# De-Rosa/PPO-BipedalWalker

Measured on NVIDIA B200. Metric: walker env-steps/sec (SAT physics step), higher is better.
Workload: dtype f32

## Files before the change

ppo-bipedalwalker_b200/csrc/physics_lanes.cu:

```cuda
#include <cstdio>
#include <cstdlib>
#include "physics.cuh"
#include "physics_math.cuh"

#ifndef WB_SAT_UNROLL
#define WB_SAT_UNROLL 6
#endif

namespace wb {
namespace pl {
constexpr int kSatUnroll = WB_SAT_UNROLL;

constexpr unsigned kFull = 0xFFFFFFFFu;

#ifdef WB_PHASE_PROFILE
__device__ unsigned long long g_prof[24];
__device__ __forceinline__ long long prof_clock() {
  long long t;
  asm volatile("mov.u64 %0, %%clock64;" : "=l"(t)::"memory");
  return t;
}
__device__ long long g_prof_sat_scratch;
#endif


__constant__ Material c_materials[WB_MAX_MATERIALS];
__constant__ float c_init_state[kStateFloats];
__constant__ FloorConst c_floor;

enum { LLL = 0, LLU = 1, BODY = 2, RLL = 3, RLU = 4, FLOOR = 5 };

constexpr int kV2Cen = 30;
constexpr int kV2Vel = 35;
constexpr int kV2Count = 40;
constexpr int kFOmega = 0;
constexpr int kFAngle = 5;
constexpr int kFCount = 10;

__device__ __forceinline__ int nverts(int b) { return b == BODY ? 5 : 6; }

template <int L_, int E_>
struct Env {
  static constexpr int L = L_;
  static constexpr int E = E_;
  float2* v2;
  float* f;
  const FloorConst* fl;
  int sub;
  int gsub;
  int gshift;
  int col;
  bool live;
  int flags;
  float im_w;
  float ii_pole;
  float e_ww, mu_ww, e_wf, mu_wf;
};

template <class EV> __device__ __forceinline__ float2& V2(const EV& e, int slot) { return e.v2[slot * EV::E]; }
template <class EV> __device__ __forceinline__ float& F1(const EV& e, int slot) { return e.f[slot * EV::E]; }
template <class EV> __device__ __forceinline__ float inv_inertia(const EV& e, int b) { return b == BODY ? 0.0003f : e.ii_pole; }
template <class EV> __device__ __forceinline__ void set_materials(EV& e, const Material& mw, const Material& mf) {
  e.im_w = mw.inverse_mass;
  e.ii_pole = fmul(0.001f, mw.inverse_mass);
  e.e_ww = net_max(mw.restitution, mw.restitution);
  e.mu_ww = net_min(mw.friction, mw.friction);
  e.e_wf = net_max(mw.restitution, mf.restitution);
  e.mu_wf = net_min(mw.friction, mf.friction);
}
template <int L> __device__ __forceinline__ void lanes_sync() { if (L > 1) __syncwarp(); }
template <class EV, int G> __device__ __forceinline__ bool group_any(const EV& e, bool pred) {
  if (EV::L == 1) return pred;
  const unsigned b = __ballot_sync(kFull, pred);
  return ((b >> e.gshift) & ((1u << G) - 1u)) != 0u;
}

struct BodyDyn {
  float2 c, v;
  float w, im, ii;
};

template <class EV> __device__ __forceinline__ BodyDyn load_dyn(const EV& e, int b) {
  BodyDyn d;
  d.c = V2(e, kV2Cen + b);
  d.v = V2(e, kV2Vel + b);
  d.w = F1(e, kFOmega + b);
  d.im = e.im_w;
  d.ii = inv_inertia(e, b);
  return d;
}
template <class EV> __device__ __forceinline__ BodyDyn floor_dyn(const EV& e) {
  BodyDyn d;
  d.c = e.fl->cen;
  d.v = mk2(0.0f, 0.0f);
  d.w = 0.0f;
  d.im = 0.0f;
  d.ii = 0.0f;
  return d;
}
template <class EV> __device__ __forceinline__ void store_dyn(const EV& e, int b, const BodyDyn& d) {
  V2(e, kV2Vel + b) = d.v;
  F1(e, kFOmega + b) = d.w;
}

__device__ __forceinline__ void calculate_impulse(const BodyDyn& A, const BodyDyn& B, float2 contact, float force, float2 n,
                                                  float2& rA, float2& rB, float& impulse) {
  rA = vsub(contact, A.c);
  const float2 perpA = mk2(-rA.y, rA.x);
  const float kA = vdot(n, perpA);
  rB = vsub(contact, B.c);
  const float2 perpB = mk2(-rB.y, rB.x);
  const float kB = vdot(n, perpB);
  const float2 va = vadd(A.v, vmul(perpA, A.w));
  const float2 vb = vadd(B.v, vmul(perpB, B.w));
  const float2 vrel = vsub(vb, va);
  const float vn = vdot(vrel, n);
  const float j = fmul(-force, vn);
  const float2 k = mk2(kA, kB);
  const float2 kki = vmul2_nosum(vmul2_nosum(k, k), mk2(A.ii, B.ii));
  const float denom = fadd(fadd(fadd(A.im, B.im), kki.x), kki.y);
  impulse = fdiv(j, denom);
}

__device__ __forceinline__ void apply_impulses(BodyDyn& A, BodyDyn& B, float2 n, float impulse, float2 rA, float2 rB) {
  const float2 J = vmul(n, impulse);
  const float2 velA = vsub(A.v, vmul(J, A.im));
  const float2 velB = vadd(B.v, vmul(J, B.im));
  const float2 perpA = mk2(-rA.y, rA.x);
  const float wA = fsub(A.w, fmul(vdot(perpA, J), A.ii));
  const float2 perpB = mk2(-rB.y, rB.x);
  const float wB = fadd(B.w, fmul(vdot(perpB, J), B.ii));
  A.v = velA;
  B.v = velB;
  A.w = wA;
  B.w = wB;
}

template <class EV, int G>
__device__ __forceinline__ void move_bodies(const EV& e, bool on, int A, float2 dA, bool moveB, int B, float2 dB) {
#pragma unroll
  for (int it0 = 0; it0 < 14; it0 += G) {
    const int it = it0 + e.gsub;
    const bool second = it >= 7;
    const int k = second ? it - 7 : it;
    const int b = second ? B : A;
    if (on && it < 14 && (!second || moveB)) {
      const int slot = (k < 6) ? b * 6 + k : kV2Cen + b;
      V2(e, slot) = vadd(V2(e, slot), second ? dB : dA);
    }
  }
}

template <class EV, bool TRACE, int G = EV::L>
__device__ __forceinline__ void joint_step(const EV& e, int A, int ia, int B, int ib, wb_joint_trace* tr) {
  const bool leader = (G == EV::L) ? e.sub == 0 : e.gsub == 0;
  const float2 pA = V2(e, A * 6 + ia);
  const float2 pB = V2(e, B * 6 + ib);
  float2 ab = vsub(pB, pA);
  const float depth = fsqrt(vdot(ab, ab));
  if (TRACE) {
    if (tr && e.live && leader) {
      tr->active = !(depth < 0.1f);
      tr->depth = depth;
    }
  }
  const bool active = e.live && !(depth < 0.1f);
  if (!__any_sync(kFull, active)) return;
  ab = vnormalize_fast(ab);
  const float2 dA = vhalf(vmul(ab, depth));
  const float2 dB = vhalf(vmul(vneg(ab), depth));
  BodyDyn X = load_dyn(e, B);
  BodyDyn Y = load_dyn(e, A);
  lanes_sync<EV::L>();
  move_bodies<EV, G>(e, active, A, dA, true, B, dB);
  X.c = vadd(X.c, dB);
  Y.c = vadd(Y.c, dA);
  const float2 contact = vhalf(vadd(vadd(pA, dA), vadd(pB, dB)));
  float2 rX, rY;
  float j;
  calculate_impulse(X, Y, contact, fadd(1.0f, 1.0f), ab, rX, rY, j);
  apply_impulses(X, Y, ab, j, rX, rY);
  if (active && leader) {
    store_dyn(e, B, X);
    store_dyn(e, A, Y);
  }
  lanes_sync<EV::L>();
}

__device__ __forceinline__ void project6(const float2 (&P)[6], float2 ax, float& mn, float& mx) {
  const float t0 = vdot(ax, P[0]), t1 = vdot(ax, P[1]), t2 = vdot(ax, P[2]);
  const float t3 = vdot(ax, P[3]), t4 = vdot(ax, P[4]), t5 = vdot(ax, P[5]);
  mn = fminf(fminf(fminf(FLT_MAX, t0), fminf(t1, t2)), fminf(fminf(t3, t4), t5));
  mx = fmaxf(fmaxf(fmaxf(-FLT_MAX, t0), fmaxf(t1, t2)), fmaxf(fmaxf(t3, t4), t5));
}
__device__ __forceinline__ void project4(const float2* P, float2 ax, float& mn, float& mx) {
  const float t0 = vdot(ax, P[0]), t1 = vdot(ax, P[1]), t2 = vdot(ax, P[2]), t3 = vdot(ax, P[3]);
  mn = fminf(fminf(fminf(FLT_MAX, t0), t1), fminf(t2, t3));
  mx = fmaxf(fmaxf(fmaxf(-FLT_MAX, t0), t1), fmaxf(t2, t3));
}

struct Face {
  float2 a, b, max;
};

__device__ __forceinline__ Face face_from(float2 sv, float2 next, float2 prev, float2 nrm) {
  const float2 after = vnormalize_fast(vsub(sv, next));
  const float2 before = vnormalize_fast(vsub(sv, prev));
  const bool use_before = vdot(nrm, before) >= vdot(nrm, after);
  Face f;
  f.a = use_before ? sv : next;
  f.b = use_before ? prev : sv;
  f.max = sv;
  return f;
}

__device__ __forceinline__ int support_index6(const float2 (&P)[6], float2 nrm) {
  float best = FLT_MAX;
  int k = 0;
#pragma unroll
  for (int i = 0; i < 6; i++) {
    const float pr = vdot(P[i], nrm);
    const bool lt = pr < best;
    k = lt ? i : k;
    best = lt ? pr : best;
  }
  return k;
}

template <class EV>
__device__ __forceinline__ Face significant_face_body(const EV& e, int b, const float2 (&P)[6], float2 nrm) {
  const int n = nverts(b);
  const int k = support_index6(P, nrm);
  const int kn = (k + 1 == n) ? 0 : k + 1;
  const int kp = (k == 0) ? n - 1 : k - 1;
  return face_from(V2(e, b * 6 + k), V2(e, b * 6 + kn), V2(e, b * 6 + kp), nrm);
}

template <class EV>
__device__ __forceinline__ Face significant_face_floor(const EV& e, float2 nrm) {
  float best = FLT_MAX;
  int k = 0;
#pragma unroll
  for (int i = 0; i < 4; i++) {
    const float pr = vdot(e.fl->v[i], nrm);
    const bool lt = pr < best;
    k = lt ? i : k;
    best = lt ? pr : best;
  }
  return face_from(e.fl->v[k], e.fl->v[(k + 1) & 3], e.fl->v[(k + 3) & 3], nrm);
}

__device__ __forceinline__ int clip_vectors(float2 a, float2 b, float2 nrm, float offset, float2& o0, float2& o1) {
  int cnt = 0;
  const float2 dab = vsub(mk2(vdot(a, nrm), vdot(b, nrm)), mk2(offset, offset));
  const float da = dab.x, db = dab.y;
  if (da >= 0.0f) {
    o0 = a;
    cnt = 1;
  }
  if (db >= 0.0f) {
    if (cnt == 0) o0 = b; else o1 = b;
    cnt++;
  }
  if (fmul(da, db) < 0.0f) {
    float2 ed = vsub(b, a);
    const float location = fdiv(da, fsub(da, db));
    ed = vmul(ed, location);
    ed = vadd(ed, a);
    if (cnt == 0) o0 = ed; else if (cnt == 1) o1 = ed;
    cnt++;
  }
  return cnt;
}

__device__ __forceinline__ bool veq(float2 a, float2 b) { return a.x == b.x && a.y == b.y; }

__device__ __forceinline__ int contact_points(Face ref, Face inc, float2 normal, float2& c0, float2& c1) {
  float2 rf = vsub(ref.b, ref.a);
  const float2 ifv = vsub(inc.b, inc.a);
  if (fabsf(vdot(rf, normal)) > fabsf(vdot(ifv, normal))) {
    const Face t = ref;
    ref = inc;
    inc = t;
    rf = vsub(ref.b, ref.a);
  }
  rf = vnormalize_fast(rf);
  float offset = vdot(rf, ref.a);
  float2 p0 = mk2(0.f, 0.f), p1 = mk2(0.f, 0.f);
  int cnt = clip_vectors(inc.a, inc.b, rf, offset, p0, p1);
  if (cnt < 2) return 0;
  offset = vdot(rf, ref.b);
  float2 q0 = mk2(0.f, 0.f), q1 = mk2(0.f, 0.f);
  cnt = clip_vectors(p0, p1, vneg(rf), -offset, q0, q1);
  if (cnt < 2) return 0;
  cnt = 2;
  const float2 rn = mk2(rf.y, -rf.x);
  const float maximum = vdot(rn, ref.max);
  if (fsub(vdot(rn, q0), maximum) < 0.0f) {
    q0 = q1;
    cnt = 1;
  }
  const float2 last = (cnt == 2) ? q1 : q0;
  if (fsub(vdot(rn, last), maximum) < 0.0f) {
    if (cnt == 2) {
      if (veq(q0, q1)) q0 = q1;
      cnt = 1;
    } else {
      cnt = 0;
    }
  }
  c0 = q0;
  c1 = q1;
  return cnt;
}

__device__ __forceinline__ void resolve_impulses(BodyDyn& X, BodyDyn& Y, int ncp, float2 c0, float2 c1, float2 normal, float e, float mu) {
  const float2 contact = (ncp == 2) ? vhalf(vadd(c0, c1)) : c0;
  const float2 tangent = mk2(-normal.y, normal.x);
  float2 rA, rB, rAf, rBf;
  float j, jf;
  calculate_impulse(X, Y, contact, fadd(1.0f, e), normal, rA, rB, j);
  calculate_impulse(X, Y, contact, mu, tangent, rAf, rBf, jf);
  apply_impulses(X, Y, normal, j, rA, rB);
  apply_impulses(X, Y, tangent, jf, rAf, rBf);
}

__device__ __forceinline__ void resolve_impulses_split(BodyDyn& X, BodyDyn& Y, int ncp, float2 c0, float2 c1, float2 normal, float e, float mu,
                                                       bool odd) {
  const float2 contact = (ncp == 2) ? vhalf(vadd(c0, c1)) : c0;
  const float2 tangent = mk2(-normal.y, normal.x);
  float2 rA, rB;
  float mine;
  calculate_impulse(X, Y, contact, odd ? mu : fadd(1.0f, e), odd ? tangent : normal, rA, rB, mine);
  const float other = __shfl_xor_sync(kFull, mine, 1);
  apply_impulses(X, Y, normal, odd ? other : mine, rA, rB);
  apply_impulses(X, Y, tangent, odd ? mine : other, rA, rB);
}

__device__ __forceinline__ void aabb6(const float2 (&P)[6], float2& mn, float2& mx) {
  mn.x = fminf(fminf(fminf(P[0].x, P[1].x), fminf(P[2].x, P[3].x)), fminf(P[4].x, P[5].x));
  mn.y = fminf(fminf(fminf(P[0].y, P[1].y), fminf(P[2].y, P[3].y)), fminf(P[4].y, P[5].y));
  mx.x = fmaxf(fmaxf(fmaxf(P[0].x, P[1].x), fmaxf(P[2].x, P[3].x)), fmaxf(P[4].x, P[5].x));
  mx.y = fmaxf(fmaxf(fmaxf(P[0].y, P[1].y), fmaxf(P[2].y, P[3].y)), fmaxf(P[4].y, P[5].y));
}
__device__ __forceinline__ bool aabb_hit(float2 amin, float2 amax, float2 bmin, float2 bmax) {
  return amin.x < bmax.x && amax.x > bmin.x && amin.y < bmax.y && amax.y > bmin.y;
}

#ifndef WB_SHARED_CONTACTS
#define WB_SHARED_CONTACTS 0
#endif
}
namespace pc {
template <int G, int kE> __device__ __forceinline__ void group_env_by_col(pl::Env<G, kE>& e, int col, bool live);
}
namespace pl {
template <class EV, int G>
__device__ __noinline__ void contact_stage_shared(int col, bool live, bool colliding, int A, int B, bool floorb, float depth, int idx, float2 normal) {
  static_assert(G > 1, "two or more lanes per pair");
  EV e;
  pc::group_env_by_col<G, EV::E>(e, col, live);
  const FloorConst& fl = *e.fl;
#pragma unroll
  for (int m = 1; m < G; m <<= 1) {
    const float od = __shfl_xor_sync(kFull, depth, m);
    const int oi = __shfl_xor_sync(kFull, idx, m);
    const float ox = __shfl_xor_sync(kFull, normal.x, m);
    const float oy = __shfl_xor_sync(kFull, normal.y, m);
    if (od < depth || (od == depth && oi < idx)) {
      depth = od;
      idx = oi;
      normal = mk2(ox, oy);
    }
  }
  BodyDyn X = load_dyn(e, A);
  BodyDyn Y = load_dyn(e, floorb ? A : B);
  if (floorb) Y = floor_dyn(e);
  if (vdot(vsub(Y.c, X.c), normal) > 0.0f) normal = vmul(normal, -1.0f);
  const bool odd = (e.gsub & 1) != 0;
  const float2 nn = odd ? vneg(normal) : normal;
  const bool mine_floor = odd && floorb;
  const float2* vb = mine_floor ? fl.v : &V2(e, (odd ? B : A) * 6);
  const int stride = mine_floor ? 1 : EV::E;
  const int n = mine_floor ? 4 : nverts(odd ? B : A);
  float2 P[6];
#pragma unroll
  for (int i = 0; i < 6; i++) P[i] = vb[((mine_floor && i >= 4) ? 0 : i) * stride];
  const int k = support_index6(P, nn);
  const int kn = (k + 1 == n) ? 0 : k + 1;
  const int kp = (k == 0) ? n - 1 : k - 1;
  const Face mine = face_from(vb[k * stride], vb[kn * stride], vb[kp * stride], nn);
  Face other;
  other.a.x = __shfl_xor_sync(kFull, mine.a.x, 1);
  other.a.y = __shfl_xor_sync(kFull, mine.a.y, 1);
  other.b.x = __shfl_xor_sync(kFull, mine.b.x, 1);
  other.b.y = __shfl_xor_sync(kFull, mine.b.y, 1);
  other.max.x = __shfl_xor_sync(kFull, mine.max.x, 1);
  other.max.y = __shfl_xor_sync(kFull, mine.max.y, 1);
  const Face ref = odd ? other : mine;
  const Face inc = odd ? mine : other;
  float2 c0 = mk2(0.f, 0.f), c1 = mk2(0.f, 0.f);
  const int ncp = contact_points(ref, inc, normal, c0, c1);
  const float2 dA = floorb ? vmul(normal, depth) : vhalf(vmul(normal, depth));
  const float2 dB = floorb ? mk2(0.f, 0.f) : vhalf(vmul(vneg(normal), depth));
  lanes_sync<EV::L>();
  move_bodies<EV, G>(e, colliding, A, dA, !floorb, B, dB);
  X.c = vadd(X.c, dA);
  if (!floorb) Y.c = vadd(Y.c, dB);
  resolve_impulses_split(X, Y, ncp, c0, c1, normal, floorb ? e.e_wf : e.e_ww, floorb ? e.mu_wf : e.mu_ww, odd);
  if (ncp > 0 && colliding && e.gsub == 0) {
    store_dyn(e, A, X);
    if (!floorb) store_dyn(e, B, Y);
  }
  lanes_sync<EV::L>();
}

template <class EV, int G, bool TRACE, bool FLOORB, int VOTE = -1, bool KNOWN_HIT = false, bool SHARED_CONTACTS = false>
__device__ __forceinline__ void resolve_pair(EV& e, bool want, int A, int B, wb_pair_trace* tr, int* sep_axis = nullptr) {
  const FloorConst& fl = *e.fl;
  float2 PA[6], PB[6];
#pragma unroll
  for (int i = 0; i < 6; i++) PA[i] = V2(e, A * 6 + i);
  if (!FLOORB) {
#pragma unroll
    for (int i = 0; i < 6; i++) PB[i] = V2(e, B * 6 + i);
  }
  bool hit = want;
  if (!KNOWN_HIT) {
    float2 amin, amax, bmin, bmax;
    aabb6(PA, amin, amax);
    if (FLOORB) {
      bmin = fl.bb_min;
      bmax = fl.bb_max;
    } else {
      aabb6(PB, bmin, bmax);
    }
    hit = want && aabb_hit(amin, amax, bmin, bmax);
  }
  if (FLOORB && hit) e.flags |= (1 << A);
  wb_pair_trace rec;
  if (TRACE) {
    rec.other = FLOORB ? FLOOR : B;
    rec.aabb = hit ? 1 : 0;
    rec.sat = 0;
    rec.axis = -1;
    rec.nx = rec.ny = rec.depth = 0.0f;
    rec.ncontacts = 0;
    rec.c0x = rec.c0y = rec.c1x = rec.c1y = 0.0f;
  }
#ifdef WB_PHASE_PROFILE
  const long long rp_t0 = prof_clock();
  long long rp_t1 = rp_t0;
#endif
  bool colliding = false;
  if (__any_sync(kFull, hit)) {
    const int nA = nverts(A);
    float depth = FLT_MAX;
    float2 normal = mk2(0.0f, 0.0f);
    int idx = 0x7FFFFFFF;
    bool sep = false;
    constexpr bool kVote = VOTE < 0 ? (G != 4) : (VOTE != 0);
    bool my_sep = false;
    auto accumulate = [&](bool use, float2 axis, int axis_idx, float omin, float omax, float tmin, float tmax) {
      const float2 dd = vsub(mk2(tmax, omax), mk2(omin, tmin));
      const float temp = fminf(dd.x, dd.y);
      const bool overlapping = (omin < tmax) && (tmin < omax);
      if (use && temp < depth) {
        depth = temp;
        normal = axis;
        idx = axis_idx;
      }
      if (sep_axis != nullptr && use && !overlapping && !sep && !my_sep) *sep_axis = axis_idx;
      if (!kVote) {
        my_sep = my_sep || (use && !overlapping);
        return false;
      }
      const bool separated = group_any<EV, G>(e, use && !overlapping);
      sep = sep || separated;
      return !__any_sync(kFull, hit && !sep);
    };
    auto edge_axis = [&](int own, int k, bool& skip) {
      const float2 p0 = V2(e, own * 6 + k), p1 = V2(e, own * 6 + (k == 5 ? 0 : k + 1));
      const float2 edge = vsub(p1, p0);
      const float2 axis = mk2(-edge.y, edge.x);
      skip = (axis.x == 0.0f) && (axis.y == 0.0f);
      return vnormalize_fast(axis);
    };
    auto edge_axis_reg = [&](const float2 (&P)[6], int r, bool odd, bool& skip) {
      const float2 p0 = odd ? P[(r + 1) % 6] : P[r % 6], p1 = odd ? P[(r + 2) % 6] : P[(r + 1) % 6];
      const float2 edge = vsub(p1, p0);
      const float2 axis = mk2(-edge.y, edge.x);
      skip = (axis.x == 0.0f) && (axis.y == 0.0f);
      return vnormalize_fast(axis);
    };
    auto round_a_vs_floor = [&](int r) {
      const int i = r + e.gsub;
      const bool valid = i < 6;
      bool skip;
      const float2 axis = (G == 2 && !kVote) ? edge_axis_reg(PA, r, e.gsub != 0, skip) : edge_axis(A, valid ? i : 0, skip);
      float omin, omax, tmin, tmax;
      project6(PA, axis, omin, omax);
      project4(fl.v, axis, tmin, tmax);
      return accumulate(valid && !skip, axis, i, omin, omax, tmin, tmax);
    };
    auto round_floor_vs_a = [&](int r) {
      const int i = r + e.gsub;
      const bool valid = i < 4;
      const int k = valid ? i : 0;
      const float2 axis = fl.axis[k];
      float tmin, tmax;
      project6(PA, axis, tmin, tmax);
      return accumulate(valid && fl.skip[k] == 0, axis, nA + k, fl.pmin[k], fl.pmax[k], tmin, tmax);
    };
    auto round_pole = [&](int r) {
      const int i = r + e.gsub;
      const bool valid = i < 12;
      const bool ownA = i < 6;
      const int k = ownA ? i : (valid ? i - 6 : 0);
      bool skip;
      float2 axis;
      if (G == 2 && !kVote) {
        axis = (r < 6) ? edge_axis_reg(PA, r, e.gsub != 0, skip) : edge_axis_reg(PB, r - 6, e.gsub != 0, skip);
      } else {
        axis = edge_axis(ownA ? A : B, k, skip);
      }
      float amn, amx, bmn, bmx;
      project6(PA, axis, amn, amx);
      project6(PB, axis, bmn, bmx);
      return accumulate(valid && !skip, axis, ownA ? i : nA + k, amn, amx, bmn, bmx);
    };
    if (kVote) {
      if (FLOORB) {
        bool done = false;
#pragma unroll 1
        for (int r = 0; r < 6 && !done; r += G) done = round_a_vs_floor(r);
#pragma unroll 1
        for (int r = 0; r < 4 && !done; r += G) done = round_floor_vs_a(r);
      } else {
#pragma unroll 1
        for (int r = 0; r < 12; r += G)
          if (round_pole(r)) break;
      }
    } else {
      if (FLOORB) {
#pragma unroll kSatUnroll
        for (int r = 0; r < 6; r += G) round_a_vs_floor(r);
#pragma unroll kSatUnroll
        for (int r = 0; r < 4; r += G) round_floor_vs_a(r);
      } else {
#pragma unroll kSatUnroll
        for (int r = 0; r < 12; r += G) round_pole(r);
      }
      sep = group_any<EV, G>(e, my_sep);
    }
    colliding = hit && !sep;
#ifdef WB_PHASE_PROFILE
    rp_t1 = prof_clock();
#endif
    if constexpr (SHARED_CONTACTS && G > 1 && !TRACE) {
      if (__any_sync(kFull, colliding)) contact_stage_shared<EV, G>(e.col, e.live, colliding, A, B, FLOORB, depth, idx, normal);
    } else if (__any_sync(kFull, colliding)) {
      if (G > 1) {
#pragma unroll
        for (int m = 1; m < G; m <<= 1) {
          const float od = __shfl_xor_sync(kFull, depth, m);
          const int oi = __shfl_xor_sync(kFull, idx, m);
          const float ox = __shfl_xor_sync(kFull, normal.x, m);
          const float oy = __shfl_xor_sync(kFull, normal.y, m);
          if (od < depth || (od == depth && oi < idx)) {
            depth = od;
            idx = oi;
            normal = mk2(ox, oy);
          }
        }
      }
      BodyDyn X = load_dyn(e, A);
      BodyDyn Y = FLOORB ? floor_dyn(e) : load_dyn(e, B);
      if (vdot(vsub(Y.c, X.c), normal) > 0.0f) normal = vmul(normal, -1.0f);
      Face ref, inc;
      if (G == 1) {
        ref = significant_face_body(e, A, PA, normal);
        inc = FLOORB ? significant_face_floor(e, vneg(normal)) : significant_face_body(e, B, PB, vneg(normal));
      } else {
        const bool odd = (e.gsub & 1) != 0;
        const float2 nn = odd ? vneg(normal) : normal;
        float2 P[6];
        int n, stride;
        const float2* vb;
        if (FLOORB) {
#pragma unroll
          for (int i = 0; i < 6; i++) {
            const float2 f = fl.v[i < 4 ? i : 0];
            P[i] = odd ? f : PA[i];
          }
          n = odd ? 4 : nA;
          vb = odd ? fl.v : &V2(e, A * 6);
          stride = odd ? 1 : EV::E;
        } else {
#pragma unroll
          for (int i = 0; i < 6; i++) P[i] = odd ? PB[i] : PA[i];
          n = nverts(odd ? B : A);
          vb = &V2(e, (odd ? B : A) * 6);
          stride = EV::E;
        }
        const int k = support_index6(P, nn);
        const int kn = (k + 1 == n) ? 0 : k + 1;
        const int kp = (k == 0) ? n - 1 : k - 1;
        const Face mine = face_from(vb[k * stride], vb[kn * stride], vb[kp * stride], nn);
        Face other;
        other.a.x = __shfl_xor_sync(kFull, mine.a.x, 1);
        other.a.y = __shfl_xor_sync(kFull, mine.a.y, 1);
        other.b.x = __shfl_xor_sync(kFull, mine.b.x, 1);
        other.b.y = __shfl_xor_sync(kFull, mine.b.y, 1);
        other.max.x = __shfl_xor_sync(kFull, mine.max.x, 1);
        other.max.y = __shfl_xor_sync(kFull, mine.max.y, 1);
        ref = odd ? other : mine;
        inc = odd ? mine : other;
      }
      float2 c0 = mk2(0.f, 0.f), c1 = mk2(0.f, 0.f);
      const int ncp = contact_points(ref, inc, normal, c0, c1);
      if (TRACE) {
        if (colliding) {
          rec.sat = 1;
          rec.axis = idx;
          rec.nx = normal.x;
          rec.ny = normal.y;
          rec.depth = depth;
          rec.ncontacts = ncp;
          if (ncp > 0) {
            rec.c0x = c0.x;
            rec.c0y = c0.y;
          }
          if (ncp > 1) {
            rec.c1x = c1.x;
            rec.c1y = c1.y;
          }
        }
      }
      const float2 dA = FLOORB ? vmul(normal, depth) : vhalf(vmul(normal, depth));
      const float2 dB = FLOORB ? mk2(0.f, 0.f) : vhalf(vmul(vneg(normal), depth));
      lanes_sync<EV::L>();
      move_bodies<EV, G>(e, colliding, A, dA, !FLOORB, B, dB);
      X.c = vadd(X.c, dA);
      if (!FLOORB) Y.c = vadd(Y.c, dB);
      if (G == 1) {
        if (ncp > 0) resolve_impulses(X, Y, ncp, c0, c1, normal, FLOORB ? e.e_wf : e.e_ww, FLOORB ? e.mu_wf : e.mu_ww);
      } else {
        resolve_impulses_split(X, Y, ncp, c0, c1, normal, FLOORB ? e.e_wf : e.e_ww, FLOORB ? e.mu_wf : e.mu_ww, (e.gsub & 1) != 0);
      }
      if (ncp > 0 && colliding && e.gsub == 0) {
        store_dyn(e, A, X);
        if (!FLOORB) store_dyn(e, B, Y);
      }
      lanes_sync<EV::L>();
    }
  }
  if (TRACE) {
    if (tr && want && e.gsub == 0) *tr = rec;
  }
#ifdef WB_PHASE_PROFILE
  const unsigned prof_want = __ballot_sync(kFull, want), prof_coll = __ballot_sync(kFull, colliding);
  if (!TRACE && (threadIdx.x & 31) == 0) {
    const long long rp_t2 = prof_clock();
    const int k = FLOORB ? 1 : 0;
    atomicAdd(&g_prof[8 + 4 * k + 0], (unsigned long long)(rp_t1 - rp_t0));
    atomicAdd(&g_prof[8 + 4 * k + 1], (unsigned long long)(rp_t2 - rp_t1));
    atomicAdd(&g_prof[8 + 4 * k + 2], 1ull);
    atomicAdd(&g_prof[8 + 4 * k + 3], (unsigned long long)__popc(prof_want) | ((unsigned long long)__popc(prof_coll) << 32));
  }
#endif
}


template <class EV, int G, bool TRACE>
__device__ __forceinline__ void body_step(EV& e, bool on, int b, float dt, wb_pair_trace* tr_base) {
  float2 v = V2(e, kV2Vel + b);
  v = vadd(v, vmul(mk2(0.0f, 980.0f), dt));
  const float2 d = vmul(v, dt);
  const float w = F1(e, kFOmega + b);
  const float theta = fmul(w, dt);
  float ang = fadd(F1(e, kFAngle + b), theta);
  const float PI_F = 3.14159274f, TAU_F = 6.28318548f;
  if (ang > PI_F) ang = fsub(ang, TAU_F);
  else if (ang < -PI_F) ang = fadd(ang, TAU_F);
  float m11, m12;
  rotz(theta, m11, m12);
  const float2 cen = vadd(V2(e, kV2Cen + b), d);
  lanes_sync<EV::L>();
#pragma unroll
  for (int i0 = 0; i0 < 6; i0 += G) {
    const int i = i0 + e.gsub;
    if (i < 6 && on) {
      float2 p = vadd(V2(e, b * 6 + i), d);
      p = vsub(p, cen);
      const float2 t = vrotate(p, m11, m12);
      V2(e, b * 6 + i) = vadd(t, cen);
    }
  }
  if (e.gsub == 0 && on) {
    V2(e, kV2Cen + b) = cen;
    V2(e, kV2Vel + b) = v;
    F1(e, kFAngle + b) = ang;
  }
  lanes_sync<EV::L>();
  const int slot = (0x75420 >> (4 * b)) & 0xF;
  const int partner = (0x34F01 >> (4 * b)) & 0xF;
  const bool floor_first = (e.flags & WB_FLAG_FLOOR_FIRST) != 0;
#pragma unroll 1
  for (int phase = 0; phase < 3; phase++) {
    if (phase == 1) {
      const bool want = on && b != BODY;
      if (__any_sync(kFull, want))
        resolve_pair<EV, G, TRACE, false>(e, want, b, b == BODY ? LLL : partner, (TRACE && tr_base) ? tr_base + slot + (floor_first ? 1 : 0) : nullptr);
    } else {
      const bool want = on && ((b == BODY) ? (phase == 0) : ((phase == 0) == floor_first));
      if (__any_sync(kFull, want))
        resolve_pair<EV, G, TRACE, true>(e, want, b, FLOOR, (TRACE && tr_base) ? tr_base + slot + ((b == BODY || floor_first) ? 0 : 1) : nullptr);
    }
  }
}

template <class EV>
__device__ __forceinline__ void store_observation(const EV& e, float* dst) {
  const float2 j0 = V2(e, BODY * 6 + 1), j2 = V2(e, LLU * 6 + 2), j3 = V2(e, RLU * 6 + 2), bv = V2(e, kV2Vel + BODY);
  float4* d4 = reinterpret_cast<float4*>(dst);
  d4[0] = make_float4(fdiv(j0.x, 900.0f), fdiv(j0.y, 500.0f), fdiv(j2.x, 900.0f), fdiv(j2.y, 500.0f));
  d4[1] = make_float4(fdiv(j3.x, 900.0f), fdiv(j3.y, 500.0f), fdiv(bv.x, 60.0f), fdiv(bv.y, 60.0f));
  d4[2] = make_float4(F1(e, kFAngle + LLL), F1(e, kFAngle + LLU), F1(e, kFAngle + RLL), F1(e, kFAngle + RLU));
}

template <int E>
__device__ __forceinline__ int record_word(int f) {
  if (f < 58) {
    const int vtx = f >> 1, slot = vtx + (vtx >= 17 ? 1 : 0);
    return slot * E * 2 + (f & 1);
  }
  if (f < 78) return (kV2Cen + ((f - 58) >> 1)) * E * 2 + (f & 1);
  return kV2Count * E * 2 + (f - 78) * E;
}

template <int L, int LEGS, bool TRACE>
__global__ void __launch_bounds__(32, (L <= 4) ? 16 : 8) physics_lanes_kernel(const PhysicsParams p) {
  static_assert(LEGS == 1 || (LEGS == 2 && L >= 2), "the leg split needs at least two lanes per environment");
  constexpr int E = 32 / L;
  __shared__ __align__(16) float s_state[(kV2Count * 2 + kFCount) * E];
  __shared__ FloorConst s_floor;
  const int lane = threadIdx.x;
  const int env0 = blockIdx.x * E;

  for (int w = lane; w < (int)(sizeof(FloorConst) / 4); w += 32)
    reinterpret_cast<uint32_t*>(&s_floor)[w] = reinterpret_cast<const uint32_t*>(&c_floor)[w];
  for (int idx = lane; idx < 88 * E; idx += 32) {
    int f, c;
    if (idx < 78 * E) {
      const int slot = idx / (2 * E), r = idx % (2 * E);
      c = r >> 1;
      f = 2 * slot + (r & 1);
    } else {
      f = 78 + (idx - 78 * E) / E;
      c = idx % E;
    }
    const int env = env0 + c;
    const float v = (env < p.n) ? p.state[state_index(f, env, p.n_pad)] : c_init_state[f];
    s_state[record_word<E>(f) + (f < 78 ? 2 * c : c)] = v;
  }
  __syncwarp();

  using EV = Env<L, E>;
  EV e;
  const int col = lane / L;
  const int env = env0 + col;
  e.v2 = reinterpret_cast<float2*>(s_state) + col;
  e.f = s_state + kV2Count * E * 2 + col;
  e.fl = &s_floor;
  e.sub = lane % L;
  e.gsub = e.sub;
  e.gshift = col * L;
  e.live = env < p.n;
  const int envc = e.live ? env : 0;
  if (e.sub == 0) V2(e, BODY * 6 + 5) = V2(e, BODY * 6);
  float* torque_rows = p.state + (size_t)88 * p.n_pad + envc;

  e.flags = p.flags[envc];
  int steps = p.steps[envc];
  {
    const Material mw = c_materials[p.walker_mat[envc]];
    const Material mf = c_materials[p.floor_mat[envc]];
    set_materials(e, mw, mf);
  }
  float2 pos = mk2(p.pos[envc], p.pos[p.n_pad + envc]);
  __syncwarp();

  auto write_initial_record = [&](bool on) {
    if (!__any_sync(kFull, on)) return;
    __syncwarp();
    if (on && e.sub == 0) {
#pragma unroll 1
      for (int f = 0; f < 88; f++) s_state[record_word<E>(f) + (f < 78 ? 2 * col : col)] = c_init_state[f];
      V2(e, BODY * 6 + 5) = V2(e, BODY * 6);
      for (int k = 0; k < 4; k++) torque_rows[(size_t)k * p.n_pad] = c_init_state[88 + k];
    }
    __syncwarp();
  };

  if (p.phases & kPhaseResetMasked) {
    const bool on = e.live && (p.reset_mask == nullptr || p.reset_mask[envc]);
    write_initial_record(on);
    if (on) {
      e.flags = (p.phases & kPhaseFirstEpisode) ? 0 : WB_FLAG_FLOOR_FIRST;
      steps = 0;
      pos = V2(e, kV2Cen + BODY);
    }
  }
  if (p.phases & kPhaseIncSteps) steps++;

  if (p.phases & kPhaseTakeActions) {
    if (e.live && e.sub == 0) {
      const float4 a4 = *reinterpret_cast<const float4*>(p.actions + (size_t)env * 4);
      const float act[4] = {a4.x, a4.y, a4.z, a4.w};
#pragma unroll
      for (int k = 0; k < 4; k++) {
        float a = act[k];
        if (a >= 1.0f) a = 1.0f;
        else if (a <= -1.0f) a = -1.0f;
        const float change = fsub(a, torque_rows[(size_t)k * p.n_pad]);
        torque_rows[(size_t)k * p.n_pad] = a;
        const int bodyB = (k == 0) ? LLU : (k == 1) ? RLU : (k == 2) ? LLL : RLL;
        F1(e, kFOmega + bodyB) = fadd(F1(e, kFOmega + bodyB), fmul(change, 5.0f));
      }
    }
    __syncwarp();
  }

  if (p.phases & kPhaseStepObjects) {
    const float dt = fdiv(p.dt, (float)p.iterations);
#pragma unroll 1
    for (int it = 0; it < p.iterations; it++) {
      wb_joint_trace* jt = nullptr;
      wb_pair_trace* pt = nullptr;
      if (TRACE) {
        if (p.joint_trace) jt = p.joint_trace + ((size_t)envc * p.iterations + it) * 4;
        if (p.pair_trace) pt = p.pair_trace + ((size_t)envc * p.iterations + it) * WB_PAIR_SLOTS;
      }
      if (LEGS == 1) {
#pragma unroll 1
        for (int k = 0; k < 4; k++) {
          const int A = (0x4122 >> (4 * k)) & 0xF, B = (0x3041 >> (4 * k)) & 0xF;
          joint_step<EV, TRACE>(e, A, k < 2 ? 1 : 2, B, k < 2 ? 4 : 3, jt ? jt + k : nullptr);
        }
      } else {
        constexpr int G = L / LEGS;
        joint_step<EV, TRACE>(e, BODY, 1, LLU, 4, jt ? jt + 0 : nullptr);
        const int leg = e.sub / G;
        e.gsub = e.sub % G;
        e.gshift = col * L + leg * G;
        const bool left = leg == 0;
        joint_step<EV, TRACE, G>(e, left ? LLU : BODY, left ? 2 : 1, left ? LLL : RLU, left ? 3 : 4, jt ? jt + (left ? 2 : 1) : nullptr);
        e.gsub = e.sub;
        e.gshift = col * L;
        joint_step<EV, TRACE>(e, RLU, 2, RLL, 3, jt ? jt + 3 : nullptr);
      }
      if (LEGS == 1) {
#pragma unroll 1
        for (int b = 0; b < 5; b++) body_step<EV, L, TRACE>(e, e.live, b, dt, pt);
      } else {
        constexpr int G = L / LEGS;
        const int leg = e.sub / G;
        e.gsub = e.sub % G;
        e.gshift = col * L + leg * G;
#pragma unroll 1
        for (int k = 0; k < 3; k++) {
          const bool on = e.live && (leg == 0 || k < 2);
          body_step<EV, G, TRACE>(e, on, leg == 0 ? k : (k < 2 ? RLL + k : RLU), dt, pt);
        }
        e.gsub = e.sub;
        e.gshift = col * L;
      }
    }
    if (LEGS == 2) e.flags |= __shfl_xor_sync(kFull, e.flags, L / LEGS);
  }

  if (p.phases & kPhaseObserve) {
    const float2 prev = pos;
    pos = V2(e, kV2Cen + BODY);
    if (e.flags & ((1 << BODY) | (1 << LLU) | (1 << RLU))) e.flags |= WB_FLAG_TERMINAL;
    const float dx = fsub(pos.x, prev.x);
    const float h = fdiv(V2(e, BODY * 6 + 1).y, 500.0f);
    float r = 0.0f;
    r = fadd(r, (dx > 0.0f && h < 1.6f) ? dx : 0.0f);
    r = fsub(r, (h > 1.65f) ? -0.1f : 0.0f);
    bool terminal = false;
    if ((e.flags & WB_FLAG_TERMINAL) || steps > p.max_timesteps) {
      if (e.flags & WB_FLAG_TERMINAL) r = fsub(r, 40.0f);
      terminal = true;
    }
    if (pos.x > 900.0f) {
      r = fadd(r, 80.0f);
      terminal = true;
    }
    const bool reset_now = e.live && terminal && (p.phases & kPhaseAutoReset);
    write_initial_record(reset_now);
    if (reset_now) {
      e.flags = WB_FLAG_FLOOR_FIRST;
      steps = 0;
      pos = V2(e, kV2Cen + BODY);
    }
    if (e.live && e.sub == 0) {
      store_observation(e, p.obs + (size_t)env * WB_OBS);
      p.reward[env] = r;
      p.done[env] = terminal ? 1 : 0;
    }
  } else if (p.phases & kPhaseObsOnly) {
    if (e.live && e.sub == 0) store_observation(e, p.obs + (size_t)env * WB_OBS);
  }

  if (e.live && e.sub == 0) {
    p.flags[env] = e.flags;
    p.steps[env] = steps;
    p.pos[env] = pos.x;
    p.pos[p.n_pad + env] = pos.y;
  }
  __syncwarp();
  for (int idx = lane; idx < 88 * E; idx += 32) {
    int f, c;
    if (idx < 78 * E) {
      const int slot = idx / (2 * E), r = idx % (2 * E);
      c = r >> 1;
      f = 2 * slot + (r & 1);
    } else {
      f = 78 + (idx - 78 * E) / E;
      c = idx % E;
    }
    if (env0 + c < p.n) p.state[state_index(f, env0 + c, p.n_pad)] = s_state[record_word<E>(f) + (f < 78 ? 2 * c : c)];
  }
}

__global__ void rcp_sqrt_check_kernel(uint32_t first, uint64_t count, unsigned long long* mismatches, uint32_t* first_bad) {
  const uint64_t stride = (uint64_t)gridDim.x * blockDim.x;
  unsigned long long bad = 0;
  for (uint64_t i = (uint64_t)blockIdx.x * blockDim.x + threadIdx.x; i < count; i += stride) {
    const uint32_t bits = first + (uint32_t)i;
    const float s = __uint_as_float(bits);
    const uint32_t a = __float_as_uint(rcp_sqrt_rn(s));
    const uint32_t b = __float_as_uint(__frcp_rn(__fsqrt_rn(s)));
    const bool both_nan = ((a & 0x7FFFFFFFu) > 0x7F800000u) && ((b & 0x7FFFFFFFu) > 0x7F800000u);
    if (a != b && !both_nan) {
      bad++;
      atomicMin(first_bad, bits);
    }
  }
  if (bad) atomicAdd(mismatches, bad);
}

__global__ void rotz_debug_kernel(const float* radians, int n, int mode, float* c_out, float* s_out) {
  const int i = blockIdx.x * blockDim.x + threadIdx.x;
  if (i >= n) return;
  float c, s;
  if (mode == 1) {
    sincos_dd_small((double)radians[i], c, s);
  } else if (mode == 2) {
    double sd, cd;
    sincos((double)radians[i], &sd, &cd);
    c = (float)cd;
    s = (float)sd;
  } else {
    rotz(radians[i], c, s);
  }
  c_out[i] = c;
  s_out[i] = s;
}

template <int L, int LEGS>
static cudaError_t launch_l(const PhysicsParams& p, bool trace, cudaStream_t stream) {
  constexpr int E = 32 / L;
  const int grid = (p.n + E - 1) / E;
  if (trace)
    physics_lanes_kernel<L, LEGS, true><<<grid, 32, 0, stream>>>(p);
  else
    physics_lanes_kernel<L, LEGS, false><<<grid, 32, 0, stream>>>(p);
  return cudaGetLastError();
}

}

namespace bulk {
__device__ __forceinline__ uint32_t smem_u32(const void* p) { return (uint32_t)__cvta_generic_to_shared(p); }
__device__ __forceinline__ void mbar_init(unsigned long long* bar, uint32_t count) {
  asm volatile("mbarrier.init.shared::cta.b64 [%0], %1;" ::"r"(smem_u32(bar)), "r"(count) : "memory");
}
__device__ __forceinline__ void fence_mbar_init() { asm volatile("fence.mbarrier_init.release.cluster;" ::: "memory"); }
__device__ __forceinline__ void mbar_expect_tx(unsigned long long* bar, uint32_t bytes) {
  asm volatile("mbarrier.arrive.expect_tx.shared::cta.b64 _, [%0], %1;" ::"r"(smem_u32(bar)), "r"(bytes) : "memory");
}
__device__ __forceinline__ void mbar_wait(unsigned long long* bar, uint32_t parity) {
  uint32_t ok = 0;
  while (!ok) {
    asm volatile(
        "{\n\t"
        ".reg .pred p;\n\t"
        "mbarrier.try_wait.parity.shared::cta.b64 p, [%1], %2;\n\t"
        "selp.b32 %0, 1, 0, p;\n\t"
        "}"
        : "=r"(ok)
        : "r"(smem_u32(bar)), "r"(parity)
        : "memory");
  }
}
__device__ __forceinline__ void load(void* smem_dst, const void* gmem_src, uint32_t bytes, unsigned long long* bar) {
  asm volatile("cp.async.bulk.shared::cluster.global.mbarrier::complete_tx::bytes [%0], [%1], %2, [%3];" ::"r"(smem_u32(smem_dst)),
               "l"(gmem_src), "r"(bytes), "r"(smem_u32(bar))
               : "memory");
}
__device__ __forceinline__ void store(void* gmem_dst, const void* smem_src, uint32_t bytes) {
  asm volatile("cp.async.bulk.global.shared::cta.bulk_group [%0], [%1], %2;" ::"l"(gmem_dst), "r"(smem_u32(smem_src)), "r"(bytes) : "memory");
}
__device__ __forceinline__ void fence_proxy_async() { asm volatile("fence.proxy.async.shared::cta;" ::: "memory"); }
__device__ __forceinline__ void commit_and_wait_reads() {
  asm volatile("cp.async.bulk.commit_group;" ::: "memory");
  asm volatile("cp.async.bulk.wait_group.read 0;" ::: "memory");
}
}

namespace pc {
using namespace pl;

#ifdef WB_PHASE_PROFILE
#define WB_PROF_DECL long long prof_t = prof_clock(); unsigned long long prof_acc[4] = {0, 0, 0, 0}; unsigned long long prof_items = 0, prof_rounds = 0
#define WB_PROF_MARK(k) do { const long long now_ = prof_clock(); prof_acc[k] += (unsigned long long)(now_ - prof_t); prof_t = now_; } while (0)
#else
#define WB_PROF_DECL
#define WB_PROF_MARK(k)
#endif

template <int kE>
struct Shared {
  float state[(kV2Count * 2 + kFCount) * kE];
  Material mtab[WB_MAX_MATERIALS];
  unsigned char wmat[kE], fmat[kE];
  FloorConst floor;
  unsigned char axis[4 * kE];
  unsigned short queue[3 * kE];
  unsigned char jq[4 * kE];
  int count[2];
  unsigned long long stage_bar;
#ifdef WB_PHASE_PROFILE
  long long prof_arrive[2][2][32];
#endif
};
extern __shared__ __align__(16) unsigned char smem_pc[];
template <int kE> __device__ __forceinline__ Shared<kE>& shm() { return *reinterpret_cast<Shared<kE>*>(smem_pc); }

template <int kE> __device__ __forceinline__ void scope_sync() {
  if (kE == 32) __syncwarp(); else __syncthreads();
}
template <int kE> __device__ __forceinline__ bool scope_any(bool pred) {
  if (kE == 32) return __any_sync(kFull, pred) != 0;
  return __syncthreads_or(pred) != 0;
}

template <int kE>
__device__ __forceinline__ void env_for_column(Env<1, kE>& e, Shared<kE>& S, int col, bool live) {
  e.v2 = reinterpret_cast<float2*>(S.state) + col;
  e.f = S.state + kV2Count * kE * 2 + col;
  e.fl = &S.floor;
  e.sub = 0;
  e.gsub = 0;
  e.gshift = 0;
  e.live = live;
  e.flags = 0;
  set_materials(e, S.mtab[S.wmat[col]], S.mtab[S.fmat[col]]);
}

template <int kE>
__device__ __forceinline__ void push(Shared<kE>& S, int parity, bool want, int item) {
  const unsigned m = __ballot_sync(kFull, want);
  if (m == 0) return;
  const int lane = threadIdx.x & 31;
  int base = 0;
  if (lane == 0) base = atomicAdd(&S.count[parity], __popc(m));
  base = __shfl_sync(kFull, base, 0);
  if (want) S.queue[base + __popc(m & ((1u << lane) - 1u))] = (unsigned short)item;
}

__device__ __forceinline__ int pair_slot(int b) { return b == LLL ? 0 : b == LLU ? 1 : b == RLL ? 2 : 3; }
__device__ __forceinline__ int partner_of(int b) { return (0x34F01 >> (4 * b)) & 0xF; }

template <int kE>
__device__ __noinline__ bool pole_pair_needs_work(int col, int A, int B) {
  Env<1, kE> e;
  env_for_column(e, shm<kE>(), col, true);
  const int cached = shm<kE>().axis[pair_slot(A) * kE + col];
  float2 PA[6], PB[6];
#pragma unroll
  for (int i = 0; i < 6; i++) PA[i] = V2(e, A * 6 + i);
#pragma unroll
  for (int i = 0; i < 6; i++) PB[i] = V2(e, B * 6 + i);
  const int own = cached < 6 ? A : B;
  const int k = cached < 6 ? cached : cached - 6;
  const float2 p0 = V2(e, own * 6 + k), p1 = V2(e, own * 6 + (k == 5 ? 0 : k + 1));
  const float2 edge = vsub(p1, p0);
  float2 axis = mk2(-edge.y, edge.x);
  const bool skip = (axis.x == 0.0f) && (axis.y == 0.0f);
  axis = vnormalize_fast(axis);
  float amn, amx, bmn, bmx;
  project6(PA, axis, amn, amx);
  project6(PB, axis, bmn, bmx);
  const bool overlapping = (amn < bmx) && (bmn < amx);
  if (!skip && !overlapping) return false;
  float2 amin, amax, bmin, bmax;
  aabb6(PA, amin, amax);
  aabb6(PB, bmin, bmax);
  return aabb_hit(amin, amax, bmin, bmax);
}

template <int kE>
__device__ __noinline__ bool floor_pair_needs_work(int col, int A) {
  Env<1, kE> e;
  env_for_column(e, shm<kE>(), col, true);
  float2 PA[6];
#pragma unroll
  for (int i = 0; i < 6; i++) PA[i] = V2(e, A * 6 + i);
  float2 amin, amax;
  aabb6(PA, amin, amax);
  return aabb_hit(amin, amax, e.fl->bb_min, e.fl->bb_max);
}

template <class EV>
__device__ __forceinline__ void integrate_body_inl(const EV& e, int b, float dt) {
  float2 v = V2(e, kV2Vel + b);
  v = vadd(v, vmul(mk2(0.0f, 980.0f), dt));
  const float2 d = vmul(v, dt);
  const float w = F1(e, kFOmega + b);
  const float theta = fmul(w, dt);
  float ang = fadd(F1(e, kFAngle + b), theta);
  const float PI_F = 3.14159274f, TAU_F = 6.28318548f;
  if (ang > PI_F) ang = fsub(ang, TAU_F);
  else if (ang < -PI_F) ang = fadd(ang, TAU_F);
  float m11, m12;
  rotz(theta, m11, m12);
  const float2 cen = vadd(V2(e, kV2Cen + b), d);
#pragma unroll
  for (int i = 0; i < 6; i++) {
    float2 p = vadd(V2(e, b * 6 + i), d);
    p = vsub(p, cen);
    const float2 t = vrotate(p, m11, m12);
    V2(e, b * 6 + i) = vadd(t, cen);
  }
  V2(e, kV2Cen + b) = cen;
  V2(e, kV2Vel + b) = v;
  F1(e, kFAngle + b) = ang;
}
template <int kE>
__device__ __noinline__ void integrate_body(int col, int b, float dt) {
  Env<1, kE> e;
  env_for_column(e, shm<kE>(), col, true);
  integrate_body_inl(e, b, dt);
}
#ifndef WB_FUSED_FLOOR_TEST
#define WB_FUSED_FLOOR_TEST 1
#endif
template <int kE>
__device__ __noinline__ bool integrate_body_floor_test(int col, int b, float dt) {
  Env<1, kE> e;
  env_for_column(e, shm<kE>(), col, true);
  float2 v = V2(e, kV2Vel + b);
  v = vadd(v, vmul(mk2(0.0f, 980.0f), dt));
  const float2 d = vmul(v, dt);
  const float w = F1(e, kFOmega + b);
  const float theta = fmul(w, dt);
  float ang = fadd(F1(e, kFAngle + b), theta);
  const float PI_F = 3.14159274f, TAU_F = 6.28318548f;
  if (ang > PI_F) ang = fsub(ang, TAU_F);
  else if (ang < -PI_F) ang = fadd(ang, TAU_F);
  float m11, m12;
  rotz(theta, m11, m12);
  const float2 cen = vadd(V2(e, kV2Cen + b), d);
// ... 597 lines not shown
```

Baseline: 11.27 million.

## Fold body integration into first leg slot of the two-leg sweep

In the two-leg lane split with at least four lanes per leg, the left leg's upper half-group now integrates the BODY while its lower half integrates the lower leg. The body floor AABB test uses shuffles of the freshly integrated vertices, and the floor collision resolve runs with a known-hit flag. This cuts the per-leg body_step loop from three serialized iterations to two, so the right-leg lanes no longer idle during the body step. Launch bounds for L==16 are raised to 16 blocks per SM, and the old path stays available behind WB_BODY_SLOT. The new ordering of body and leg collisions may change results, and the extra shuffles and branches add overhead.

Measured after the change: 11.95 million (median of 6 runs). 6.0% higher.

```diff
diff --git a/ppo-bipedalwalker_b200/csrc/physics_lanes.cu b/ppo-bipedalwalker_b200/csrc/physics_lanes.cu
--- a/ppo-bipedalwalker_b200/csrc/physics_lanes.cu
+++ b/ppo-bipedalwalker_b200/csrc/physics_lanes.cu
@@ -5,6 +5,9 @@
 
 #ifndef WB_SAT_UNROLL
 #define WB_SAT_UNROLL 6
+#endif
+#ifndef WB_BODY_SLOT
+#define WB_BODY_SLOT 0
 #endif
 
 namespace wb {
@@ -415,6 +418,18 @@
   lanes_sync<EV::L>();
 }
 
+__device__ __forceinline__ wb_pair_trace pair_trace_no_sat(int other, bool aabb) {
+  wb_pair_trace rec;
+  rec.other = other;
+  rec.aabb = aabb ? 1 : 0;
+  rec.sat = 0;
+  rec.axis = -1;
+  rec.nx = rec.ny = rec.depth = 0.0f;
+  rec.ncontacts = 0;
+  rec.c0x = rec.c0y = rec.c1x = rec.c1y = 0.0f;
+  return rec;
+}
+
 template <class EV, int G, bool TRACE, bool FLOORB, int VOTE = -1, bool KNOWN_HIT = false, bool SHARED_CONTACTS = false>
 __device__ __forceinline__ void resolve_pair(EV& e, bool want, int A, int B, wb_pair_trace* tr, int* sep_axis = nullptr) {
   const FloorConst& fl = *e.fl;
@@ -439,15 +454,7 @@
   }
   if (FLOORB && hit) e.flags |= (1 << A);
   wb_pair_trace rec;
-  if (TRACE) {
-    rec.other = FLOORB ? FLOOR : B;
-    rec.aabb = hit ? 1 : 0;
-    rec.sat = 0;
-    rec.axis = -1;
-    rec.nx = rec.ny = rec.depth = 0.0f;
-    rec.ncontacts = 0;
-    rec.c0x = rec.c0y = rec.c1x = rec.c1y = 0.0f;
-  }
+  if (TRACE) rec = pair_trace_no_sat(FLOORB ? FLOOR : B, hit);
 #ifdef WB_PHASE_PROFILE
   const long long rp_t0 = prof_clock();
   long long rp_t1 = rp_t0;
@@ -672,8 +679,8 @@
 }
 
 
-template <class EV, int G, bool TRACE>
-__device__ __forceinline__ void body_step(EV& e, bool on, int b, float dt, wb_pair_trace* tr_base) {
+template <class EV, int R>
+__device__ __forceinline__ void integrate_step(const EV& e, bool on, int b, int q, int nq, float dt, float2 (&P)[R]) {
   float2 v = V2(e, kV2Vel + b);
   v = vadd(v, vmul(mk2(0.0f, 980.0f), dt));
   const float2 d = vmul(v, dt);
@@ -688,21 +695,27 @@
   const float2 cen = vadd(V2(e, kV2Cen + b), d);
   lanes_sync<EV::L>();
 #pragma unroll
-  for (int i0 = 0; i0 < 6; i0 += G) {
-    const int i = i0 + e.gsub;
+  for (int r = 0; r < R; r++) {
+    const int i = r * nq + q;
+    P[r] = mk2(0.0f, 0.0f);
     if (i < 6 && on) {
       float2 p = vadd(V2(e, b * 6 + i), d);
       p = vsub(p, cen);
       const float2 t = vrotate(p, m11, m12);
-      V2(e, b * 6 + i) = vadd(t, cen);
-    }
-  }
-  if (e.gsub == 0 && on) {
+      P[r] = vadd(t, cen);
+      V2(e, b * 6 + i) = P[r];
+    }
+  }
+  if (q == 0 && on) {
     V2(e, kV2Cen + b) = cen;
     V2(e, kV2Vel + b) = v;
     F1(e, kFAngle + b) = ang;
   }
   lanes_sync<EV::L>();
+}
+
+template <class EV, int G, bool TRACE>
+__device__ __forceinline__ void resolve_candidates(EV& e, bool on, int b, wb_pair_trace* tr_base) {
   const int slot = (0x75420 >> (4 * b)) & 0xF;
   const int partner = (0x34F01 >> (4 * b)) & 0xF;
   const bool floor_first = (e.flags & WB_FLAG_FLOOR_FIRST) != 0;
@@ -720,6 +733,47 @@
   }
 }
 
+template <class EV, int G, bool TRACE>
+__device__ __forceinline__ void body_step(EV& e, bool on, int b, float dt, wb_pair_trace* tr_base) {
+  float2 P[(6 + G - 1) / G];
+  integrate_step(e, on, b, e.gsub, G, dt, P);
+  resolve_candidates<EV, G, TRACE>(e, on, b, tr_base);
+}
+
+template <class EV, int G, bool TRACE>
+__device__ __forceinline__ void legs_sweep(EV& e, bool left, float dt, wb_pair_trace* tr_base) {
+  static_assert(G >= 4, "two or more lanes per body in slot 0");
+  constexpr int H = G / 2;
+  constexpr int R = (6 + H - 1) / H;
+  const int base = e.gshift - (left ? 0 : G);
+#pragma unroll 1
+  for (int k = 0; k < 2; k++) {
+    const bool body_lane = k == 0 && left && e.gsub >= H;
+    const int seg = left ? (k == 0 ? LLL : LLU) : (k == 0 ? RLL : RLU);
+    float2 P[R];
+    integrate_step(e, e.live, body_lane ? BODY : seg, body_lane ? e.gsub - H : e.gsub, (k == 0 && left) ? H : G, dt, P);
+    if (k == 0) {
+      float2 Q[6];
+#pragma unroll
+      for (int i = 0; i < 6; i++) {
+        Q[i].x = __shfl_sync(kFull, P[i / H].x, base + H + i % H);
+        Q[i].y = __shfl_sync(kFull, P[i / H].y, base + H + i % H);
+      }
+      float2 mn, mx;
+      aabb6(Q, mn, mx);
+      const unsigned hits = __ballot_sync(kFull, body_lane && e.live && aabb_hit(mn, mx, e.fl->bb_min, e.fl->bb_max));
+      const bool body_hit = ((hits >> base) & ((1u << G) - 1u)) != 0u;
+      if (body_hit) e.flags |= 1 << BODY;
+      wb_pair_trace* tr = (TRACE && tr_base) ? tr_base + 4 : nullptr;
+      if (TRACE) {
+        if (tr && e.live && left && e.gsub == 0 && !body_hit) *tr = pair_trace_no_sat(FLOOR, false);
+      }
+      if (hits != 0u) resolve_pair<EV, G, TRACE, true, -1, true>(e, left && body_hit, left ? BODY : RLL, FLOOR, tr);
+    }
+    resolve_candidates<EV, G, TRACE>(e, e.live, seg, tr_base);
+  }
+}
+
 template <class EV>
 __device__ __forceinline__ void store_observation(const EV& e, float* dst) {
   const float2 j0 = V2(e, BODY * 6 + 1), j2 = V2(e, LLU * 6 + 2), j3 = V2(e, RLU * 6 + 2), bv = V2(e, kV2Vel + BODY);
@@ -740,7 +794,7 @@
 }
 
 template <int L, int LEGS, bool TRACE>
-__global__ void __launch_bounds__(32, (L <= 4) ? 16 : 8) physics_lanes_kernel(const PhysicsParams p) {
+__global__ void __launch_bounds__(32, (L <= 4 || L == 16) ? 16 : 8) physics_lanes_kernel(const PhysicsParams p) {
   static_assert(LEGS == 1 || (LEGS == 2 && L >= 2), "the leg split needs at least two lanes per environment");
   constexpr int E = 32 / L;
   __shared__ __align__(16) float s_state[(kV2Count * 2 + kFCount) * E];
@@ -868,10 +922,14 @@
         const int leg = e.sub / G;
         e.gsub = e.sub % G;
         e.gshift = col * L + leg * G;
-#pragma unroll 1
-        for (int k = 0; k < 3; k++) {
-          const bool on = e.live && (leg == 0 || k < 2);
-          body_step<EV, G, TRACE>(e, on, leg == 0 ? k : (k < 2 ? RLL + k : RLU), dt, pt);
+        if constexpr (G >= 4 && !WB_BODY_SLOT) {
+          legs_sweep<EV, G, TRACE>(e, leg == 0, dt, pt);
+        } else {
+#pragma unroll 1
+          for (int k = 0; k < 3; k++) {
+            const bool on = e.live && (leg == 0 || k < 2);
+            body_step<EV, G, TRACE>(e, on, leg == 0 ? k : (k < 2 ? RLL + k : RLU), dt, pt);
+          }
         }
         e.gsub = e.sub;
         e.gshift = col * L;
```
